# Scuttie/Few-Shot-Prompt-Learning-for-Vision-Language-Models-in-Imbalanced-Datasets

Hardware: AMD Instinct MI355X
Metric: CoCoOp ViT-B/16 16-shot train-step images/sec at 1/2/4/8 GPUs; eval images/sec (higher is better)
Workload: dtype fp32s

## Files before the change

few-shot-prompt-learning-for-vision-language-models-in-imbalanced-datasets_amd/_native.py:

```python
from __future__ import annotations

import ctypes
import hashlib
import os
import sys

_PKG = os.path.dirname(os.path.abspath(__file__))
LIB_PATH = os.environ.get("CLIPK_LIB") or os.path.join(_PKG, "libclipk.so")
_ROOT = os.path.dirname(_PKG)


def source_files():
    csrc = os.path.join(_PKG, "csrc")
    names = sorted(n for n in os.listdir(csrc) if n.endswith((".hip", ".h")) or n == "Makefile")
    rel = [("csrc/" + n, os.path.join(csrc, n)) for n in names]
    return rel + [("include/clipk.h", os.path.join(_ROOT, "include", "clipk.h"))]


def source_digest():
    h = hashlib.sha256()
    for rel, path in source_files():
        with open(path, "rb") as f:
            h.update(f"{hashlib.sha256(f.read()).hexdigest()}  {rel}\n".encode())
    return h.hexdigest()

F32, F16, BF16, F32S = 0, 1, 2, 3
PREFIX_CLS_GROUP0 = 1
PREFIX_SPLIT = 2
PREFIX_OUT_SPLIT = 4
F32S16 = 4
SPLIT_SCALE = 64.0
EPI_BIAS, EPI_BIAS_RES, EPI_BIAS_QGELU, EPI_DQGELU, EPI_NONE = 0, 1, 2, 3, 4
A_QGELU = 0x100
QGELU_DERIV = 0x200
OUT_SPLIT, A_SPLIT = 0x400, 0x800
ADAM_ADAM, ADAM_ADAMW, ADAM_AMSGRAD = 0, 1, 2
PROF_NONE, PROF_GEMM_FC, PROF_GEMM_ALL, PROF_ATTN, PROF_LN, PROF_GEMM_DGELU = 0, 1, 2, 3, 4, 5

_P = ctypes.c_void_p
_I = ctypes.c_int
_L = ctypes.c_long
_F = ctypes.c_float
_S = ctypes.c_size_t
_D = ctypes.c_double
_U = ctypes.c_uint

SIGNATURES = {
    "clipk_version": (ctypes.c_char_p, []),
    "clipk_source_digest": (ctypes.c_char_p, []),
    "clipk_strerror": (ctypes.c_char_p, [_I]),
    "clipk_device_arch_ok": (_I, []),
    "clipk_gemm": (_I, [_I, _I, _I, _I, _I, _I, _P, _I, _P, _I, _P, _P, _I, _P, _I, _P, _P, _I, _I, _P]),
    "clipk_gemm_auto_splits": (_I, [_I, _I, _I, _I]),
    "clipk_gemm_splitk_ws_bytes": (_S, [_I, _I, _I]),
    "clipk_gemm_splitk": (_I, [_I, _I, _I, _I, _I, _I, _P, _I, _P, _I, _P, _P, _I, _P, _I, _P, _I, _P, _S, _P]),
    "clipk_gemm_set_config": (_I, [_I]),
    "clipk_split_pack": (_I, [_I, _I, _P, _I, _P, _P]),
    "clipk_split_lo_zero": (_I, [_I, _I, _P, _P, _P]),
    "clipk_split_hi16": (_I, [_I, _I, _P, _P, _P]),
    "clipk_gemm_ln": (_I, [_I, _I, _I, _I, _I, _P, _I, _P, _I, _P, _P, _I, _P, _I, _P, _P, _P, _P, _P]),
    "clipk_ln_stats_merge": (_I, [_I, _I, _P, _P, _P, _P, _P]),
    "clipk_gemm_ln_merge_fused": (_I, [_I, _I, _I, _I]),
    "clipk_gemm_split_tile_rows": (_I, [_I, _I, _I, _I, _I]),
    "clipk_gemm_t256_cost": (_D, [_I, _I, _I]),
    "clipk_gemm_ln_stats_split": (_I, [_I, _I, _I, _I, _I, _P, _I, _P, _I, _P, _P, _I, _P, _I, _P, _P, _P, _P]),
    "clipk_gemm_ln_gamma": (_I, [_I, _I, _I, _I, _I, _P, _I, _P, _I, _P, _P, _I, _P, _P, _P, _P, _P]),
    "clipk_gemm_ln_merge": (_I, [_I, _I, _I, _I, _I, _P, _I, _P, _I, _P, _P, _I, _P, _P, _P, _P, _P, _P, _P]),
    "clipk_image_resample": (_I, [_I, _I, _I, _P, _P, _P, _P, _P, _P, _I, _P, _P]),
    "clipk_gemm_stamps": (_I, [_P, _S]),
    "clipk_layernorm_fwd": (_I, [_I, _I, _I, _P, _I, _P, _P, _P, _P, _I, _P, _P, _P]),
    "clipk_layernorm_bwd": (_I, [_I, _I, _I, _P, _I, _P, _I, _P, _P, _P, _P, _P, _I, _P, _P, _I, _P, _I, _P]),
    "clipk_layernorm_fwd_x": (_I, [_I, _I, _I, _I, _P, _I, _P, _P, _P, _P, _I, _P, _P, _P]),
    "clipk_layernorm_bwd_x": (_I, [_I, _I, _I, _I, _P, _I, _P, _I, _P, _P, _P, _P, _P, _I, _P, _P, _I, _P, _I, _P]),
    "clipk_layernorm_bwd_x2": (_I, [_I, _I, _I, _I, _P, _I, _P, _I, _P, _P, _P, _P, _P, _I, _I, _P, _P, _I, _P, _I, _P]),
    "clipk_attention_fwd": (_I, [_I, _I, _I, _I, _I, _P, _I, _P, _I, _P, _P]),
    "clipk_attention_bwd": (_I, [_I, _I, _I, _I, _I, _I, _P, _I, _P, _I, _P, _I, _P, _P, _I, _P]),
    "clipk_im2col": (_I, [_I, _I, _I, _I, _I, _P, _P, _P]),
    "clipk_vit_embed_ln": (_I, [_I, _I, _I, _P, _P, _P, _P, _P, _P, _P]),
    "clipk_prompt_assemble": (_I, [_I, _I, _I, _I, _P, _P, _P, _L, _L, _P, _P, _P, _P]),
    "clipk_ctx_grad": (_I, [_I, _I, _I, _I, _I, _I, _P, _P, _P, _P]),
    "clipk_prompt_assemble_rows": (_I, [_I, _I, _I, _I, _I, _P, _P, _P, _P, _L, _L, _P, _P, _P, _P]),
    "clipk_ctx_grad_rows": (_I, [_I, _I, _I, _I, _P, _P, _P, _P, _P]),
    "clipk_ctx_bias_grad_rows": (_I, [_I, _I, _I, _I, _P, _P, _P, _P, _P, _P]),
    "clipk_attention_prefix_fwd": (_I, [_I, _I, _I, _I, _I, _P, _P, _I, _P, _I, _P, _I, _P, _P]),
    "clipk_attention_prefix_ws_bytes": (_S, [_I, _I, _I]),
    "clipk_attention_prefix_bwd": (_I, [_I, _I, _I, _I, _I, _I, _P, _P, _I, _P, _I, _P, _I, _P, _I, _P, _P,
                                        _I, _P, _S, _P]),
    "clipk_attention_prefix_fwd_ex": (_I, [_I, _I, _I, _I, _I, _P, _P, _I, _P, _I, _P, _I, _P, _I, _P]),
    "clipk_attention_prefix_bwd_ex": (_I, [_I, _I, _I, _I, _I, _I, _P, _P, _I, _P, _I, _P, _I, _P, _I, _P, _P,
                                           _I, _P, _S, _I, _P]),
    "clipk_cosine_logits_fwd": (_I, [_I, _I, _I, _I, _F, _P, _P, _P, _P, _P, _P]),
    "clipk_cosine_logits_bwd": (_I, [_I, _I, _I, _I, _F, _P, _P, _P, _P, _P, _P, _P]),
    "clipk_ce_loss": (_I, [_I, _I, _P, _P, _P, _F, _I, _F, _P, _P, _P]),
    "clipk_ce_loss_reduce": (_I, [_I, _I, _P, _P, _P, _F, _I, _F, _I, _P, _P, _P, _P]),
    "clipk_ce_loss_mix": (_I, [_I, _I, _P, _P, _P, _F, _P, _F, _I, _F, _I, _P, _P, _P, _P]),
    "clipk_mixup_images": (_I, [_I, _L, _P, _P, _P, _P, _F, _F, _P, _P]),
    "clipk_ntxent_ws_bytes": (_S, [_I, _I]),
    "clipk_ntxent_loss": (_I, [_I, _I, _P, _P, _F, _F, _P, _P, _P, _P, _P]),
# ... 123 lines not shown
```

few-shot-prompt-learning-for-vision-language-models-in-imbalanced-datasets_amd/csrc/attention.hip:

```cpp
#include "attn_common.h"

namespace clipk {

template <int LP, typename T>
__global__ __launch_bounds__(256) void attn_fwd_short(int nseq, int L, int H, int causal,
                                                      const T* __restrict__ qkv, int ldq,
                                                      T* __restrict__ out, int ldo,
                                                      float* __restrict__ lse) {
  constexpr int G = 64 / LP;
  constexpr int V = Vec16<T>::N;
  __shared__ CLIPK_LDS_ALIGN T sk[4][64 * 64];
  __shared__ CLIPK_LDS_ALIGN T sv[4][64 * 64];
  const int lane = threadIdx.x & 63, w = threadIdx.x >> 6;
  const int g = lane / LP, i = lane % LP;
  const int pair = (blockIdx.x * 4 + w) * G + g;
  const bool pair_ok = pair < nseq * H;
  const int s = pair_ok ? pair / H : 0, h = pair_ok ? pair % H : 0;
  const int W = H * 64;
  const bool row_ok = pair_ok && i < L;
  const size_t row = (size_t)s * L + (row_ok ? i : 0);
  const T* qp = qkv + row * ldq + h * 64;

  T* myk = &sk[w][lane * 64];
  T* myv = &sv[w][lane * 64];
// ... 416 lines not shown
      t8 pv;
#pragma unroll
      for (int j = 0; j < 8; ++j) pv[j] = (T)p[j];
      const s16x8 pb = __builtin_bit_cast(s16x8, pv);
#pragma unroll
      for (int t = 0; t < 4; ++t) {
        const s16x4 lo = tr_read(sV, kb + 4 * g4, 16 * t, lane), hi = tr_read(sV, kb + 16 + 4 * g4, 16 * t, lane);
        const s16x8 va = __builtin_shufflevector(lo, hi, 0, 1, 2, 3, 4, 5, 6, 7);
        o[t] = mfma32_t<T>(va, pb, o[t]);
      }
    }
  }
  const float lt = xsum4(l);
  const float inv = 1.0f / lt;
  if (qok) {
    T* op = out + (row0 + qr) * ldo + h * 64 + 4 * g4;
#pragma unroll
    for (int t = 0; t < 4; ++t)
      *reinterpret_cast<s16x4*>(op + 16 * t) = pack4<T>(o[t][0] * inv, o[t][1] * inv, o[t][2] * inv, o[t][3] * inv);
    if (lse && g4 == 0) lse[(row0 + qr) * H + h] = (m + __log2f(lt)) * 0.6931471805599453f;
  }
}

template <typename T, typename TG>
__device__ __forceinline__ float row_D(const TG* dor, const T* orow, bool ok, int g4) {
  float acc = 0.f;
  if (ok) {
#pragma unroll
    for (int kk = 0; kk < 2; ++kk) {
      float a[8], b[8];
      load16_f32<TG>(dor + 8 * g4 + 32 * kk, a);
      load16_f32<T>(orow + 8 * g4 + 32 * kk, b);
#pragma unroll
      for (int c = 0; c < 8; ++c) acc = fmaf(a[c], b[c], acc);
    }
  }
  acc += __shfl_xor(acc, 16, 64);
  acc += __shfl_xor(acc, 32, 64);
  return acc;
}

template <typename T, typename TG>
__global__ __launch_bounds__(256) void attn_bwd_long_kv(int nseq, int L, int H, int causal,
                                                        const T* __restrict__ qkv, int ldq,
                                                        const T* __restrict__ o_fwd, int ldof,
                                                        const TG* __restrict__ dout, int lddo,
// ... 347 lines not shown
    CLIPK_CHECK_LAUNCH();
    return CLIPK_OK;
  }
  auto go = [&](auto lp_tag) {
    constexpr int LP = decltype(lp_tag)::value;
    constexpr int G = 64 / LP;
    const int blocks = (pairs + G - 1) / G;
    hipLaunchKernelGGL((attn_bwd_short<LP, T, TG>), dim3(blocks), dim3(64), 0, st, nseq, L, H,
                       causal, (const T*)qkv, ldq, (const T*)ofwd, ldof, (const TG*)dout, lddo, lse,
                       (TG*)dqkv, lddq);
  };
  if (L <= 16) go(std::integral_constant<int, 16>{});
  else if (L <= 32) go(std::integral_constant<int, 32>{});
  else if (L <= 64) go(std::integral_constant<int, 64>{});
  else return CLIPK_ESHAPE;
  CLIPK_CHECK_LAUNCH();
  return CLIPK_OK;
}

}

using namespace clipk;

extern "C" int clipk_attention_fwd(int dtype, int nseq, int L, int heads, int causal,
                                   const void* qkv, int ldqkv, void* out, int ldo, float* lse,
                                   void* stream) {
  if (!qkv || !out) return CLIPK_EINVAL;
  if (nseq < 0 || L <= 0 || heads <= 0 || ldqkv < 3 * heads * 64 || ldo < heads * 64 || ldqkv % 8 ||
      ldo % 8)
    return CLIPK_ESHAPE;
  if (nseq == 0) return CLIPK_OK;
  hipStream_t st = (hipStream_t)stream;
  switch (dtype) {
    case CLIPK_F16: return launch_fwd<f16>(nseq, L, heads, causal, qkv, ldqkv, out, ldo, lse, st);
    case CLIPK_BF16: return launch_fwd<bf16>(nseq, L, heads, causal, qkv, ldqkv, out, ldo, lse, st);
    case CLIPK_F32: return launch_fwd<float>(nseq, L, heads, causal, qkv, ldqkv, out, ldo, lse, st);
    default: return CLIPK_EDTYPE;
  }
}

extern "C" int clipk_attention_bwd(int dtype, int grad_dtype, int nseq, int L, int heads,
                                    int causal, const void* qkv, int ldqkv, const void* ofwd,
                                    int ldof, const void* dout, int lddo, const float* lse,
                                    void* dqkv, int lddqkv, void* stream) {
  if (!qkv || !ofwd || !dout || !lse || !dqkv) return CLIPK_EINVAL;
  if (nseq < 0 || L <= 0 || heads <= 0 || ldqkv < 3 * heads * 64 || lddqkv < 3 * heads * 64 ||
      ldof < heads * 64 || lddo < heads * 64)
    return CLIPK_ESHAPE;
  if (nseq == 0) return CLIPK_OK;
  hipStream_t st = (hipStream_t)stream;
#define CLIPK_BWD(TT, TGG) \
  return launch_bwd<TT, TGG>(nseq, L, heads, causal, qkv, ldqkv, ofwd, ldof, dout, lddo, lse, dqkv, lddqkv, st)
  if (dtype == CLIPK_F16 && grad_dtype == CLIPK_BF16) CLIPK_BWD(f16, bf16);
  if (dtype == CLIPK_F16 && grad_dtype == CLIPK_F16) CLIPK_BWD(f16, f16);
  if (dtype == CLIPK_BF16 && grad_dtype == CLIPK_BF16) CLIPK_BWD(bf16, bf16);
  if (dtype == CLIPK_F32 && grad_dtype == CLIPK_F32) CLIPK_BWD(float, float);
#undef CLIPK_BWD
  return CLIPK_EDTYPE;
}
```

few-shot-prompt-learning-for-vision-language-models-in-imbalanced-datasets_amd/csrc/attention_prefix.hip:

```cpp
#include <cstdlib>

#include "attn_common.h"

namespace clipk {

constexpr int kValuChunkMin = 4;

static int chunk_env(const char* name, int def) {
  const char* e = getenv(name);
  const int v = e ? atoi(e) : def;
  return v >= 1 && v <= 16 ? v : def;
}
static int lds_slots();
static int fwd_chunk() { static int c = chunk_env("CLIPK_PREFIX_FWD_CHUNK", lds_slots() ? 4 : 8); return c; }
static int bwd_chunk() { static int c = chunk_env("CLIPK_PREFIX_BWD_CHUNK", 16); return c; }
static int prefix_num_cus() {
  static int n = 0;
  if (!n) {
    int dev = 0, v = 0;
    n = (hipGetDevice(&dev) == hipSuccess &&
         hipDeviceGetAttribute(&v, hipDeviceAttributeMultiprocessorCount, dev) == hipSuccess && v > 0)
            ? v
            : 256;
  }
// ... 919 lines not shown
          akp[d] = fmaf(dsp, a[d], akp[d]);
          avp[d] = fmaf(pp, b[d], avp[d]);
        }
      }
      if (qok) {
        if constexpr (OS) {
          st16x_split(dqkv + row * lddq + W + h * 64 + kSl * s, dk, s);
          st16x_split(dqkv + row * lddq + 2 * W + h * 64 + kSl * s, dv, s);
        } else {
          st16x(dqkv + row * lddq + W + h * 64 + kSl * s, dk);
          st16x(dqkv + row * lddq + 2 * W + h * 64 + kSl * s, dv);
        }
      }
    }
    lds_sync();
  }
  if (r < P) {
    float* pb = part + (((size_t)g * nchunk + k) * 16 + r) * (2 * W) + h * 64 + kSl * s;
    st16x(pb, akp);
    st16x(pb + W, avp);
  }
}

constexpr float kPScale = 4096.0f, kPInv = 1.0f / 4096.0f;

struct Parts8 { s16x8 hi[2], lo[2]; };

__device__ __forceinline__ void ld_frag32(const float* p, f32x4 (&x)[4]) {
#pragma unroll
  for (int i = 0; i < 4; ++i) x[i] = *reinterpret_cast<const f32x4*>(p + 16 * i);
}
__device__ __forceinline__ void split_frag(const f32x4 (&x)[4], Parts8& o) {
#pragma unroll
  for (int kk = 0; kk < 2; ++kk) {
    f16x8 h, l;
#pragma unroll
    for (int j = 0; j < 2; ++j)
#pragma unroll
      for (int e = 0; e < 4; ++e) {
        const float v = x[2 * kk + j][e];
        const f16 hh = (f16)v;
        h[4 * j + e] = hh;
        l[4 * j + e] = (f16)(v - (float)hh);
      }
    o.hi[kk] = __builtin_bit_cast(s16x8, h);
    o.lo[kk] = __builtin_bit_cast(s16x8, l);
  }
}
__device__ __forceinline__ void split_pack4(float a, float b, float c, float d, s16x4& hi, s16x4& lo) {
  float x[4] = {a, b, c, d};
  typedef f16 h4 __attribute__((ext_vector_type(4)));
  h4 h, l;
#pragma unroll
  for (int e = 0; e < 4; ++e) {
    asm volatile("" : "+v"(x[e]));
    h[e] = (f16)x[e];
    l[e] = (f16)(x[e] - (float)h[e]);
  }
  hi = __builtin_bit_cast(s16x4, h);
  lo = __builtin_bit_cast(s16x4, l);
}
__device__ __forceinline__ void st_parts(const Parts8& f, short* thi, short* tlo, int r16, int g4) {
#pragma unroll
  for (int i = 0; i < 4; ++i) {
    const int o = r16 * TRS + 16 * i + 4 * g4;
    const s16x8 h = f.hi[i >> 1], l = f.lo[i >> 1];
    const int b = 4 * (i & 1);
    *reinterpret_cast<s16x4*>(thi + o) = (s16x4){h[b], h[b + 1], h[b + 2], h[b + 3]};
    *reinterpret_cast<s16x4*>(tlo + o) = (s16x4){l[b], l[b + 1], l[b + 2], l[b + 3]};
  }
}
__device__ __forceinline__ f32x4 mfma32_s3(const Parts8& a, const Parts8& b, f32x4 c) {
#pragma unroll
  for (int kk = 0; kk < 2; ++kk) {
    c = mfma32_t<f16>(a.lo[kk], b.hi[kk], c);
    c = mfma32_t<f16>(a.hi[kk], b.lo[kk], c);
  }
#pragma unroll
  for (int kk = 0; kk < 2; ++kk) c = mfma32_t<f16>(a.hi[kk], b.hi[kk], c);
  return c;
}
__device__ __forceinline__ f32x4 mfma16_s3(s16x4 ah, s16x4 al, s16x4 bh, s16x4 bl, f32x4 c) {
  c = mfma16_t<f16>(al, bh, c);
  c = mfma16_t<f16>(ah, bl, c);
  return mfma16_t<f16>(ah, bh, c);
}
__device__ __forceinline__ void ld_prefix_parts(const float* p, bool ok, Parts8& o) {
  f32x4 x[4];
  ld_frag32(p, x);
#pragma unroll
  for (int i = 0; i < 4; ++i)
    if (!ok) x[i] = (f32x4){0.f, 0.f, 0.f, 0.f};
  split_frag(x, o);
}
template <bool OS>
__device__ __forceinline__ void store_acc16(float* rowp, const f32x4 v, int t, bool ok, int g4) {
  if constexpr (!OS) {
    if (ok) *reinterpret_cast<f32x4*>(rowp + 16 * t + 4 * g4) = v;
  } else {
    typedef uint32_t u32x2 __attribute__((ext_vector_type(2)));
    s16x4 h, l;
    split_pack4(v[0], v[1], v[2], v[3], h, l);
    const u32x2 hu = __builtin_bit_cast(u32x2, h), lu = __builtin_bit_cast(u32x2, l);
    const auto s0 = __builtin_amdgcn_permlane16_swap(hu[0], lu[0], false, false);
    const auto s1 = __builtin_amdgcn_permlane16_swap(hu[1], lu[1], false, false);
    if (ok)
      reinterpret_cast<u32x4*>(rowp + 16 * t + 8 * (g4 >> 1))[g4 & 1] =
          (u32x4){(uint32_t)s0[0], (uint32_t)s1[0], (uint32_t)s0[1], (uint32_t)s1[1]};
  }
}
template <bool OS>
__device__ __forceinline__ void store_acc64(float* rowp, const f32x4 (&a)[4], float scale, bool ok, int g4) {
#pragma unroll
  for (int t = 0; t < 4; ++t) store_acc16<OS>(rowp, a[t] * scale, t, ok, g4);
}

constexpr int kSplitFwdWpc = 12, kSplitBwdWpc = 8;

template <int WPB, bool OS>
__global__ __launch_bounds__(WPB * 64) void attn_prefix_fwd_split(
    int G, int P, int R, int ntiles, const int* __restrict__ tiles, const int* __restrict__ row_first, int H,
    int nchunk, int uc, const float* __restrict__ qkv, int ldq, float* __restrict__ out, int ldo,
    float* __restrict__ lse, int cls0) {
  __shared__ CLIPK_LDS_ALIGN short sm[WPB][4][16 * TRS];
  const int lane = threadIdx.x & 63, w = threadIdx.x >> 6;
  const int r16 = lane & 15, g4 = lane >> 4;
  const int wid = blockIdx.x * WPB + w;
  if (wid >= G * nchunk * H) return;
  const int h = wid % H, k = (wid / H) % nchunk, g = wid / (H * nchunk);
  const int W = H * 64;
  short* sVpH = sm[w][0];
  short* sVpL = sm[w][1];
  short* sVoH = sm[w][2];
  short* sVoL = sm[w][3];
  const size_t gR = (size_t)g * R;
  const float* qh = qkv + h * 64 + 4 * g4;
  const int u_begin = k * uc, u_end = min((k + 1) * uc, ntiles + 1);
  const int tab = load_tile_table(tiles, ntiles, u_begin, lane);

// ... 572 lines not shown
```

few-shot-prompt-learning-for-vision-language-models-in-imbalanced-datasets_amd/csrc/attn_common.h:

```cpp
#pragma once
#include "common.h"

namespace clipk {

constexpr float kScale = 0.125f;
typedef uint32_t u32x4 __attribute__((ext_vector_type(4)));

template <typename T>
__device__ __forceinline__ void load_row64(const T* p, float* out) {
  constexpr int V = Vec16<T>::N;
#pragma unroll
  for (int c = 0; c < 64 / V; ++c) load16_f32<T>(p + c * V, out + c * V);
}

template <typename T>
__device__ __forceinline__ void store_row64(T* p, const float* in) {
  constexpr int V = Vec16<T>::N;
#pragma unroll
  for (int c = 0; c < 64 / V; ++c) store16_f32<T>(p + c * V, in + c * V);
}

template <typename T>
__device__ __forceinline__ void load_cols8(const T* p, float* out) {
  constexpr int V = Vec16<T>::N;
// ... 192 lines not shown
#pragma unroll
  for (int s = 0; s < 4; s += 2)
#pragma unroll
    for (int dw = 0; dw < 2; ++dw) {
      const auto r = __builtin_amdgcn_permlane32_swap(d[s][dw], d[s + 1][dw], false, false);
      d[s][dw] = r[0];
      d[s + 1][dw] = r[1];
    }
#pragma unroll
  for (int s = 0; s < 4; s += 2)
#pragma unroll
    for (int dw = 0; dw < 2; ++dw) {
      const auto r = __builtin_amdgcn_permlane16_swap(d[s][dw], d[s + 1][dw], false, false);
      d[s][dw] = r[0];
      d[s + 1][dw] = r[1];
    }
  if (ok) {
    const int g4 = (threadIdx.x & 63) >> 4;
    *reinterpret_cast<u32x4*>(rowp + 8 * g4) = (u32x4){d[0][0], d[0][1], d[1][0], d[1][1]};
    *reinterpret_cast<u32x4*>(rowp + 32 + 8 * g4) = (u32x4){d[2][0], d[2][1], d[3][0], d[3][1]};
  }
}

}
```

few-shot-prompt-learning-for-vision-language-models-in-imbalanced-datasets_amd/csrc/encoder.hip:

```cpp
#include <vector>
#include <array>
#include <cstring>
#include <new>
#include <cstdlib>
#include <algorithm>

#include "common.h"

struct DeepPrompts {
  int n_deep = 0, n_ctx = 0, n_per = 0;
  const int* rows = nullptr;
  const float* prompts = nullptr;
  float* grads = nullptr;
};

struct clipk_encoder {
  int kind;
  int W, layers, heads, E, act, grad;
  int res, patch, Kp, Limg;
  std::vector<std::array<const void*, 16>> lw;
  std::array<const void*, 8> head;
  DeepPrompts deep;
  int prefix_input = 0;
  std::vector<std::array<const void*, 6>> fold;
// ... 291 lines not shown
    SeqShape s;
    s.rows = nseq * L; s.nout = nseq; s.nseq = nseq; s.L = L; s.causal = causal;
    return s;
  }
  static SeqShape prefix(int G, int C, int P, int R, int ntiles, const int* tiles, const int* row_first) {
    SeqShape s;
    s.rows = G * R; s.nout = G * C; s.packed = true; s.causal = 1;
    s.G = G; s.C = C; s.P = P; s.R = R; s.ntiles = ntiles; s.tiles = tiles; s.row_first = row_first;
    return s;
  }
  size_t part_bytes(int heads) const { return packed ? clipk_attention_prefix_ws_bytes(G, ntiles, heads) : 0; }
};

constexpr int kPrefixSplitFwd = 1, kPrefixSplitBwd = 2, kPrefixSplitDefault = kPrefixSplitFwd | kPrefixSplitBwd;
static int prefix_split_flag(const clipk_encoder* e, int dir) {
  const char* s = getenv("CLIPK_PREFIX_SPLIT_ATTN");
  const int on = s ? atoi(s) : kPrefixSplitDefault;
  return (on & dir) && e->split != 0 && e->act == CLIPK_F32 ? CLIPK_PREFIX_SPLIT : 0;
}
static bool prefix_split_bwd(const clipk_encoder* e, const SeqShape& sh, int gd) {
  return sh.packed && gd == CLIPK_F32 && prefix_split_flag(e, kPrefixSplitBwd) != 0;
}

static int attn_fwd(const clipk_encoder* e, const SeqShape& sh, const void* qkv, void* o, float* lse,
                    hipStream_t st, int pflags = 0) {
  const int W = e->W;
  if (sh.packed)
    return clipk_attention_prefix_fwd_ex(e->act, sh.G, sh.P, sh.R, sh.ntiles, sh.tiles, sh.row_first, e->heads,
                                         qkv, 3 * W, o, W, lse,
                                         pflags | prefix_split_flag(e, kPrefixSplitFwd) |
                                             (t_osplit ? CLIPK_PREFIX_OUT_SPLIT : 0), st);
  return clipk_attention_fwd(e->act, sh.nseq, sh.L, e->heads, sh.causal, qkv, 3 * W, o, W, lse, st);
}

static int attn_bwd(const clipk_encoder* e, const SeqShape& sh, const void* qkv, const void* o,
                    const void* dout, const float* lse, void* dqkv, void* part, hipStream_t st,
                    bool dqkv_split = false, int pflags = 0) {
  const int W = e->W;
  if (sh.packed)
    return clipk_attention_prefix_bwd_ex(e->act, dqkv_split ? CLIPK_F32S : e->grad, sh.G, sh.P, sh.R, sh.ntiles, sh.tiles, sh.row_first,
                                      e->heads, qkv, 3 * W, o, W, dout, W, lse, dqkv, 3 * W, part,
                                      sh.part_bytes(e->heads),
                                      pflags | (prefix_split_bwd(e, sh, e->grad) ? CLIPK_PREFIX_SPLIT : 0), st);
  return clipk_attention_bwd(e->act, e->grad, sh.nseq, sh.L, e->heads, sh.causal, qkv, 3 * W, o, W, dout, W,
                             lse, dqkv, 3 * W, st);
}

static int block_attn(const clipk_encoder* e, const std::array<const void*, 16>& w, const SeqShape& sh, int rd,
                      const void* X, void* xn, void* qkv, void* o, float* lse, float* m1, float* r1,
                      hipStream_t st, bool text, void* sk, size_t skb) {
  const int pg = text ? CLIPK_PROF_GEMM_ALL : CLIPK_PROF_NONE;
  const int W = e->W, rows = sh.rows, act = e->act;
  const double lnb = (double)rows * W * (esize(rd) + esize(act)) + (m1 ? 8.0 * rows : 0.0);
  {
    ProfScope ps(CLIPK_PROF_NONE, st, 0.0, text ? "text.ln_fwd" : "vit.ln_fwd", lnb);
// ... 54 lines not shown
static int gemm_ln(int act, int epi, int M, int N, int K, const void* A, const void* B, const float* bias,
                   const void* res, void* o, void* o2, float* stats, const float* colsum, const float* rnb,
                   hipStream_t st, int prof_cls, const char* site, const float* gamma = nullptr) {
  const double b = gemm_bytes(act, act, epi, M, N, K, o2 != nullptr, act) + (stats ? (double)M * (N / 64) * 8 : 0.0) +
                   (rnb ? 8.0 * M : 0.0) + (gamma ? 4.0 * K : 0.0);
  ProfScope ps(prof_cls, st, 2.0 * M * N * K, site, b);
  if (t_split && act == CLIPK_F32) act = t_split == 2 ? CLIPK_F32S16 : CLIPK_F32S;
  if (gamma) return clipk_gemm_ln_gamma(act, epi, M, N, K, A, K, B, K, bias, o, N, o2, colsum, rnb, gamma, st);
  return clipk_gemm_ln(act, epi, M, N, K, A, K, B, K, bias, res, N, o, N, o2, stats, colsum, rnb, st);
}
static int gemm_ln_split2(int epi, int M, int N, int K, const void* A, const void* B, const float* bias,
                          const void* res, void* o, float* stats, const float* gamma, void* xs, hipStream_t st,
                          int prof_cls, const char* site) {
  const double b = gemm_bytes(CLIPK_F32S16, CLIPK_F32, epi, M, N, K, false, CLIPK_F32) + (double)M * (N / 64) * 8 +
                   4.0 * M * N + 4.0 * N;
  ProfScope ps(prof_cls, st, 2.0 * M * N * K, site, b);
  return clipk_gemm_ln_stats_split(CLIPK_F32S16, epi, M, N, K, A, K, B, K, bias, res, N, o, N, stats, gamma, xs, st);
}
static bool ps_fold(const clipk_encoder* e) { return t_split == 2 && e->split == 2 && presplit_on(); }
static bool o_split_on(const clipk_encoder* e, const SeqShape& sh, bool fold) {
  const char* s = getenv("CLIPK_PRESPLIT_O");
  return (s ? atoi(s) != 0 : true) && fold && ps_fold(e) && sh.packed && e->lora.rank == 0 &&
         prefix_split_flag(e, kPrefixSplitFwd) != 0 && prefix_split_bwd(e, sh, e->grad);
}
static int ln_merge(int rows, int W, const float* lnst, float* m, float* r, float* rnb, hipStream_t st, bool text) {
  ProfScope ps(CLIPK_PROF_NONE, st, 0.0, text ? "text.ln_stats" : "vit.ln_stats", (double)rows * (W / 64) * 8 + 16.0 * rows);
  return clipk_ln_stats_merge(rows, W, lnst, m, r, rnb, st);
}
static int gemm_ln_merged(int act, int epi, int M, int N, int K, const void* A, const void* B, const float* bias,
                          void* o, void* o2, const float* lnst, const float* colsum, float* m, float* r,
                          float* rnb, hipStream_t st, int prof_cls, const char* site, bool text,
                          const float* gamma = nullptr) {
  if (t_split || act == CLIPK_F32 || !clipk_gemm_ln_merge_fused(act, M, N, K)) {
    TRY(ln_merge(M, K, lnst, m, r, rnb, st, text));
    return gemm_ln(act, epi, M, N, K, A, B, bias, nullptr, o, o2, nullptr, colsum, rnb, st, prof_cls, site, gamma);
  }
  const double b = gemm_bytes(act, act, epi, M, N, K, o2 != nullptr, act) + (double)M * (K / 64) * 8 + 16.0 * M;
  ProfScope ps(prof_cls, st, 2.0 * M * N * K, site, b);
  return clipk_gemm_ln_merge(act, epi, M, N, K, A, K, B, K, bias, o, N, o2, lnst, colsum, m, r, rnb, st);
}
static int block_attn_fold(const clipk_encoder* e, const std::array<const void*, 6>& f, const SeqShape& sh,
                           const void* X, void* qkv, void* o, float* lse, float* m1, float* r1, const float* lnst,
                           float* rnb, hipStream_t st, bool text, const float* gamma = nullptr,
                           const void* xs = nullptr) {
  const int W = e->W, rows = sh.rows, act = e->act;
  TRY(gemm_ln_merged(act, CLIPK_EPI_BIAS | (xs ? CLIPK_A_SPLIT : 0), rows, 3 * W, W, xs ? xs : X, f[0],
// ... 226 lines not shown
}

static int text_forward_impl(const clipk_encoder* e, const SeqShape& sh, const float* x0, const int* eot_rows,
                             float* txt, void* saved, size_t saved_bytes, void* ws, size_t ws_bytes,
                             hipStream_t st, const EncIO& io) {
  SplitScope split_scope(e);
  const bool save = saved != nullptr;
  TextBufs t = text_layout(e, sh.rows, sh.nout, saved, ws, save, io.rd);
  if (ws_bytes < t.ws_bytes || (save && saved_bytes < t.saved_bytes)) return CLIPK_EWORKSPACE;
  const int W = e->W, rows = sh.rows, rd = io.rd;
  const int pg = io.text ? CLIPK_PROF_GEMM_ALL : CLIPK_PROF_NONE;
  const void* cur = x0;
  if (save || rd != CLIPK_F32) {
    if (rd == CLIPK_F32) {
      TRY(clipk_rows_copy(W * 4, rows, x0, nullptr, t.X[0], nullptr, st));
    } else {
      TRY(clipk_cast(rd, (long)rows * W, x0, t.X[0], st));
    }
    cur = t.X[0];
  }
  const bool eotl = text_eot_last(sh);
  const int nl = e->layers, nout = sh.nout;
  const bool fold = ln_fold_on(e, io);
  t_osplit = io.text && o_split_on(e, sh, fold);
  if (save) e->o_saved_split = t_osplit;
  bool have_stats = false;
  bool xs_ready = false;
  for (int l = 0; l < nl; ++l) {
    void* Xo = t.X[l + 1];
    if (!save && Xo == cur) Xo = t.X[l];
    if (l >= 1) TRY(deep_inject(e, l, rd, const_cast<void*>(cur), st));
    const bool share0 = l == 0 && io.text && sh.G >= 2 && prefix_mode(e, sh);
    float* m1 = save ? t.mean1[l] : t.tm;
    float* r1 = save ? t.rstd1[l] : t.tr;
    float* m2 = save ? t.mean2[l] : t.tm;
    float* r2 = save ? t.rstd2[l] : t.tr;
    if (share0)
      TRY(block_attn_shared0(e, e->lw[l], sh, rd, cur, t.xn, t.qkv[l], t.o[l], t.lse[l], t.mean1[l], t.rstd1[l],
                             (int*)t.g, st));
    else if (fold && have_stats)
      TRY(block_attn_fold(e, e->fold[l], sh, cur, t.qkv[l], t.o[l], t.lse[l], m1, r1, t.lnst, t.rnb, st, io.text,
                          e->split == 2 ? (const float*)e->lw[l][0] : nullptr, xs_ready ? t.xn : nullptr));
    else
      TRY(block_attn(e, e->lw[l], sh, rd, cur, t.xn, t.qkv[l], t.o[l], t.lse[l], t.mean1[l], t.rstd1[l], st,
                     io.text, io.sk, io.skb));
    const bool compact = eotl && l == nl - 1;
    const void* xin = cur;
// ... 664 lines not shown
```

few-shot-prompt-learning-for-vision-language-models-in-imbalanced-datasets_amd/ops.py:

```python
from __future__ import annotations

import ctypes

import torch

from . import _native as N

DT = {torch.float32: N.F32, torch.float16: N.F16, torch.bfloat16: N.BF16}


def _stream():
    return ctypes.c_void_p(torch.cuda.current_stream().cuda_stream)


def _p(t):
    return None if t is None else ctypes.c_void_p(t.data_ptr())


def _need(t, name, dtype=None, cuda=True):
    if t is None:
        raise N.ClipkError(f"{name} is required")
    if cuda and not t.is_cuda:
        raise N.ClipkError(f"{name} must be a CUDA(HIP) tensor; no CPU path exists")
    if dtype is not None and t.dtype != dtype:
# ... 179 lines not shown
    _need(dy, "dy")
    R, W = dy.shape
    dx = torch.empty(R, W, device=dy.device, dtype=torch.float32)
    split = lp_dtype == "split"
    lp = (torch.empty(R, W, device=dy.device, dtype=torch.float32 if split else lp_dtype)
          if lp_dtype is not None else None)
    lpd = N.F32S if split else (DT[lp_dtype] if lp_dtype is not None else 0)
    _need(x, "x")
    N.call("clipk_layernorm_bwd_x", DT[x.dtype], DT[dy.dtype], R, W, _p(dy), W, _p(x), W, None, _p(w), _p(mean),
           _p(rstd), _p(dres), W, _p(dx), _p(lp), lpd, None, W, _stream())
    return (dx, lp) if lp is not None else dx


def layernorm_bwd_lp_(dy, x, w, mean, rstd, dres_lp, dx=None):
    _need(dy, "dy")
    _need(x, "x")
    _need(dres_lp, "dres_lp")
    R, W = dy.shape
    N.call("clipk_layernorm_bwd_x2", DT[x.dtype], DT[dy.dtype], R, W, _p(dy), W, _p(x), W, None, _p(w), _p(mean),
           _p(rstd), _p(dres_lp), DT[dres_lp.dtype], W, _p(dx), _p(dres_lp), DT[dres_lp.dtype], None, W, _stream())
    return dres_lp


def attention(qkv, nseq, L, heads, causal, lse=False):
    _need(qkv, "qkv")
    W = heads * 64
    out = torch.empty(nseq * L, W, device=qkv.device, dtype=qkv.dtype)
    l = torch.empty(nseq * L, heads, device=qkv.device) if lse else None
    N.call("clipk_attention_fwd", DT[qkv.dtype], nseq, L, heads, int(causal), _p(qkv), 3 * W, _p(out),
           W, _p(l), _stream())
    return (out, l) if lse else out


def attention_bwd(qkv, o, dout, lse, nseq, L, heads, causal, grad_dtype):
    W = heads * 64
    dqkv = torch.empty(nseq * L, 3 * W, device=qkv.device, dtype=grad_dtype)
    N.call("clipk_attention_bwd", DT[qkv.dtype], DT[grad_dtype], nseq, L, heads, int(causal), _p(qkv),
           3 * W, _p(o), W, _p(dout), W, _p(lse), _p(dqkv), 3 * W, _stream())
    return dqkv


def im2col(img, patch, Kp, out_dtype):
    _need(img, "image", torch.float32)
    B, _, R, _ = img.shape
    G = R // patch
    out = torch.empty(B * G * G, Kp, device=img.device, dtype=out_dtype)
    N.call("clipk_im2col", DT[out_dtype], B, R, patch, Kp, _p(img), _p(out), _stream())
    return out


def prompt_assemble(B, C, L, src_map, emb, ctx, ctx_sb, ctx_sc, bias, pos):
    W = emb.shape[-1]
    x0 = torch.empty(B * C * L, W, device=emb.device, dtype=torch.float32)
# ... 455 lines not shown
```

include/clipk.h:

```cpp
#ifndef CLIPK_H
#define CLIPK_H

#include <stddef.h>
#include <stdint.h>

#ifdef __cplusplus
extern "C" {
#endif

enum { CLIPK_F32 = 0, CLIPK_F16 = 1, CLIPK_BF16 = 2, CLIPK_F32S = 3, CLIPK_F32S16 = 4 };

enum {
  CLIPK_OK = 0,
  CLIPK_EINVAL = -1,
  CLIPK_ESHAPE = -2,
  CLIPK_EDTYPE = -3,
  CLIPK_EWORKSPACE = -4,
  CLIPK_ERANGE = -5,
  CLIPK_EHIP = -6
};

enum {
  CLIPK_EPI_BIAS = 0,
  CLIPK_EPI_BIAS_RES = 1,
// ... 68 lines not shown
                        const int* in_rows, const float* gamma, const float* beta,
                        void* out, int ldo, float* mean, float* rstd, void* stream);
int clipk_layernorm_fwd_x(int x_dtype, int out_dtype, int rows, int width, const void* x, int ldx,
                          const int* in_rows, const float* gamma, const float* beta,
                          void* out, int ldo, float* mean, float* rstd, void* stream);

int clipk_layernorm_bwd(int dy_dtype, int rows, int width, const void* dy, int lddy, const float* x, int ldx,
                        const int* x_rows, const float* gamma, const float* mean, const float* rstd,
                        const float* dres, int lddres, float* dx, void* dx_lp, int lp_dtype,
                        const int* out_rows, int ldo, void* stream);
int clipk_layernorm_bwd_x(int x_dtype, int dy_dtype, int rows, int width, const void* dy, int lddy,
                          const void* x, int ldx, const int* x_rows, const float* gamma,
                          const float* mean, const float* rstd, const float* dres, int lddres,
                          float* dx, void* dx_lp, int lp_dtype, const int* out_rows, int ldo,
                          void* stream);
int clipk_layernorm_bwd_x2(int x_dtype, int dy_dtype, int rows, int width, const void* dy, int lddy,
                           const void* x, int ldx, const int* x_rows, const float* gamma,
                           const float* mean, const float* rstd, const void* dres, int dres_dtype,
                           int lddres, float* dx, void* dx_lp, int lp_dtype, const int* out_rows,
                           int ldo, void* stream);

int clipk_attention_fwd(int dtype, int nseq, int L, int heads, int causal,
                        const void* qkv, int ldqkv, void* out, int ldo, float* lse, void* stream);

int clipk_attention_bwd(int dtype, int grad_dtype, int nseq, int L, int heads, int causal,
                        const void* qkv, int ldqkv, const void* ofwd, int ldof, const void* dout,
                        int lddo, const float* lse, void* dqkv, int lddqkv, void* stream);

int clipk_attention_prefix_fwd(int dtype, int G, int P, int R, int ntiles, const int* tiles,
                               const int* row_first, int heads, const void* qkv, int ldqkv, void* out,
                               int ldo, float* lse, void* stream);
size_t clipk_attention_prefix_ws_bytes(int G, int ntiles, int heads);
int clipk_attention_prefix_bwd(int dtype, int grad_dtype, int G, int P, int R, int ntiles,
                               const int* tiles, const int* row_first, int heads, const void* qkv,
                               int ldqkv, const void* ofwd, int ldof, const void* dout, int lddo,
                               const float* lse, void* dqkv, int lddqkv, void* ws, size_t ws_bytes,
                               void* stream);

enum { CLIPK_PREFIX_CLS_GROUP0 = 1, CLIPK_PREFIX_SPLIT = 2, CLIPK_PREFIX_OUT_SPLIT = 4 };
int clipk_attention_prefix_fwd_ex(int dtype, int G, int P, int R, int ntiles, const int* tiles,
                                  const int* row_first, int heads, const void* qkv, int ldqkv, void* out,
                                  int ldo, float* lse, int flags, void* stream);
int clipk_attention_prefix_bwd_ex(int dtype, int grad_dtype, int G, int P, int R, int ntiles,
                                  const int* tiles, const int* row_first, int heads, const void* qkv,
                                  int ldqkv, const void* ofwd, int ldof, const void* dout, int lddo,
                                  const float* lse, void* dqkv, int lddqkv, void* ws, size_t ws_bytes,
// ... 185 lines not shown
```

Before: 381.2.

## Add split-fp16 MFMA forward attention kernel for fp32 ViT encoder

Adds an fp32 attention forward kernel that splits Q, K, V and P into fp16 hi/lo parts and uses three fp16 MFMAs per product, replacing the fp32 path for the vision encoder when split mode is active. It can optionally write the output already split into hi/lo form, so the following out-projection GEMM can skip its own split step in non-saving passes. The aim is to move ViT attention onto matrix cores while keeping near-fp32 accuracy. The cost is extra MFMA work and some loss of precision relative to true fp32.

```diff
diff --git a/few-shot-prompt-learning-for-vision-language-models-in-imbalanced-datasets_amd/_native.py b/few-shot-prompt-learning-for-vision-language-models-in-imbalanced-datasets_amd/_native.py
--- a/few-shot-prompt-learning-for-vision-language-models-in-imbalanced-datasets_amd/_native.py
+++ b/few-shot-prompt-learning-for-vision-language-models-in-imbalanced-datasets_amd/_native.py
@@ -28,6 +28,8 @@
 PREFIX_CLS_GROUP0 = 1
 PREFIX_SPLIT = 2
 PREFIX_OUT_SPLIT = 4
+ATTN_SPLIT = 1
+ATTN_OUT_SPLIT = 2
 F32S16 = 4
 SPLIT_SCALE = 64.0
 EPI_BIAS, EPI_BIAS_RES, EPI_BIAS_QGELU, EPI_DQGELU, EPI_NONE = 0, 1, 2, 3, 4
@@ -74,6 +76,7 @@
     "clipk_layernorm_bwd_x": (_I, [_I, _I, _I, _I, _P, _I, _P, _I, _P, _P, _P, _P, _P, _I, _P, _P, _I, _P, _I, _P]),
     "clipk_layernorm_bwd_x2": (_I, [_I, _I, _I, _I, _P, _I, _P, _I, _P, _P, _P, _P, _P, _I, _I, _P, _P, _I, _P, _I, _P]),
     "clipk_attention_fwd": (_I, [_I, _I, _I, _I, _I, _P, _I, _P, _I, _P, _P]),
+    "clipk_attention_fwd_ex": (_I, [_I, _I, _I, _I, _I, _P, _I, _P, _I, _P, _I, _P]),
     "clipk_attention_bwd": (_I, [_I, _I, _I, _I, _I, _I, _P, _I, _P, _I, _P, _I, _P, _P, _I, _P]),
     "clipk_im2col": (_I, [_I, _I, _I, _I, _I, _P, _P, _P]),
     "clipk_vit_embed_ln": (_I, [_I, _I, _I, _P, _P, _P, _P, _P, _P, _P]),
diff --git a/few-shot-prompt-learning-for-vision-language-models-in-imbalanced-datasets_amd/csrc/attention.hip b/few-shot-prompt-learning-for-vision-language-models-in-imbalanced-datasets_amd/csrc/attention.hip
--- a/few-shot-prompt-learning-for-vision-language-models-in-imbalanced-datasets_amd/csrc/attention.hip
+++ b/few-shot-prompt-learning-for-vision-language-models-in-imbalanced-datasets_amd/csrc/attention.hip
@@ -462,6 +462,162 @@
   }
 }
 
+template <bool OS>
+__global__ __launch_bounds__(256) void attn_fwd_split(int nseq, int L, int H, int causal,
+                                                      const float* __restrict__ qkv, int ldq,
+                                                      float* __restrict__ out, int ldo,
+                                                      float* __restrict__ lse) {
+  __shared__ CLIPK_LDS_ALIGN short sKh[64 * TRS];
+  __shared__ CLIPK_LDS_ALIGN short sKl[64 * TRS];
+  __shared__ CLIPK_LDS_ALIGN short sVh[64 * TRS];
+  __shared__ CLIPK_LDS_ALIGN short sVl[64 * TRS];
+  constexpr float kLog2e = 1.4426950408889634f;
+  const int tid = threadIdx.x, lane = tid & 63, w = tid >> 6;
+  const int r16 = lane & 15, g4 = lane >> 4;
+  const int h = blockIdx.y, s = blockIdx.z;
+  const int W = H * 64;
+  const size_t row0 = (size_t)s * L;
+  const int q0 = blockIdx.x * 64 + w * 16;
+  const int qr = q0 + r16;
+  const bool qok = qr < L;
+  s16x8 qh[2], ql[2];
+  {
+    const float* qp = qkv + (row0 + (qok ? qr : 0)) * ldq + h * 64 + 8 * g4;
+#pragma unroll
+    for (int kk = 0; kk < 2; ++kk) {
+      f32x4 x[2];
+#pragma unroll
+      for (int c = 0; c < 2; ++c)
+        x[c] = qok ? *reinterpret_cast<const f32x4*>(qp + 32 * kk + 4 * c) : (f32x4){0.f, 0.f, 0.f, 0.f};
+      f16x8 hh, ll;
+#pragma unroll
+      for (int c = 0; c < 2; ++c)
+#pragma unroll
+        for (int e = 0; e < 4; ++e) {
+          f16 ph, pl;
+          split_parts(x[c][e] * kScale, ph, pl);
+          hh[4 * c + e] = ph;
+          ll[4 * c + e] = pl;
+        }
+      qh[kk] = __builtin_bit_cast(s16x8, hh);
+      ql[kk] = __builtin_bit_cast(s16x8, ll);
+    }
+  }
+
+  f32x4 o[4];
+#pragma unroll
+  for (int t = 0; t < 4; ++t) o[t] = (f32x4){0.f, 0.f, 0.f, 0.f};
+  float m = -INFINITY, l = 0.f;
+  const int qmax = min(L, (int)(blockIdx.x + 1) * 64) - 1;
+  const int kend = causal ? qmax + 1 : L;
+  f32x4 rk[2][2], rv[2][2];
+  auto fetch = [&](int k0) {
+#pragma unroll
+    for (int it = 0; it < 2; ++it) {
+      const int kr = k0 + it * 32 + (tid >> 3), ch = tid & 7;
+      const bool ok = kr < L;
+      const float* base = qkv + (row0 + (ok ? kr : 0)) * ldq + h * 64 + ch * 8;
+#pragma unroll
+      for (int c = 0; c < 2; ++c) {
+        rk[it][c] = ok ? *reinterpret_cast<const f32x4*>(base + W + 4 * c) : (f32x4){0.f, 0.f, 0.f, 0.f};
+        rv[it][c] = ok ? *reinterpret_cast<const f32x4*>(base + 2 * W + 4 * c) : (f32x4){0.f, 0.f, 0.f, 0.f};
+      }
+    }
+  };
+  auto st_split = [&](const f32x4& a, const f32x4& b, short* thi, short* tlo) {
+    const unsigned h01 = __builtin_bit_cast(unsigned, (f16x2){(f16)a[0], (f16)a[1]});
+    const unsigned h23 = __builtin_bit_cast(unsigned, (f16x2){(f16)a[2], (f16)a[3]});
+    const unsigned h45 = __builtin_bit_cast(unsigned, (f16x2){(f16)b[0], (f16)b[1]});
+    const unsigned h67 = __builtin_bit_cast(unsigned, (f16x2){(f16)b[2], (f16)b[3]});
+    unsigned l01, l23, l45, l67;
+    split_lo4(a[0], a[1], a[2], a[3], h01, h23, l01, l23);
+    split_lo4(b[0], b[1], b[2], b[3], h45, h67, l45, l67);
+    *reinterpret_cast<u32x4*>(thi) = (u32x4){h01, h23, h45, h67};
+    *reinterpret_cast<u32x4*>(tlo) = (u32x4){l01, l23, l45, l67};
+  };
+  fetch(0);
+  for (int k0 = 0; k0 < kend; k0 += 64) {
+    __syncthreads();
+#pragma unroll
+    for (int it = 0; it < 2; ++it) {
+      const int off = (it * 32 + (tid >> 3)) * TRS + (tid & 7) * 8;
+      st_split(rk[it][0], rk[it][1], sKh + off, sKl + off);
+      st_split(rv[it][0], rv[it][1], sVh + off, sVl + off);
+    }
+    __syncthreads();
+    if (k0 + 64 < kend) fetch(k0 + 64);
+    const int npair = min(2, (kend - k0 + 31) / 32);
+    for (int pc = 0; pc < npair; ++pc) {
+      const int kb = pc * 32;
+      const int kabs = k0 + kb;
+      if (causal && kabs > q0 + 15) break;
+      float sv[8];
+#pragma unroll
+      for (int sub = 0; sub < 2; ++sub) {
+        f32x4 sb = {0.f, 0.f, 0.f, 0.f}, ss = {0.f, 0.f, 0.f, 0.f};
+#pragma unroll
+        for (int kk = 0; kk < 2; ++kk) {
+          const int off = (kb + sub * 16 + r16) * TRS + 8 * g4 + 32 * kk;
+          const s16x8 kh = *reinterpret_cast<const s16x8*>(sKh + off);
+          const s16x8 kl = *reinterpret_cast<const s16x8*>(sKl + off);
+          ss = mfma32_t<f16>(kl, qh[kk], ss);
+          ss = mfma32_t<f16>(kh, ql[kk], ss);
+          sb = mfma32_t<f16>(kh, qh[kk], sb);
+        }
+#pragma unroll
+        for (int r = 0; r < 4; ++r) sv[4 * sub + r] = (sb[r] + ss[r]) * kLog2e;
+      }
+      if (kabs + 32 > L || (causal && kabs + 31 > q0)) {
+#pragma unroll
+        for (int j = 0; j < 8; ++j) {
+          const int key = kabs + (j < 4 ? 4 * g4 + j : 16 + 4 * g4 + j - 4);
+          if (key >= L || (causal && key > qr)) sv[j] = -INFINITY;
+        }
+      }
+      float mx = sv[0];
+#pragma unroll
+      for (int j = 1; j < 8; ++j) mx = fmaxf(mx, sv[j]);
+      mx = xmax4(mx);
+      const float mn = fmaxf(m, mx);
+      const float msafe = mn == -INFINITY ? 0.f : mn;
+      float p[8], ps = 0.f;
+#pragma unroll
+      for (int j = 0; j < 8; ++j) {
+        p[j] = __builtin_amdgcn_exp2f(sv[j] - msafe);
+        ps += p[j];
+      }
+      if (__builtin_amdgcn_ballot_w64(mn > m) != 0) {
+        const float corr = __builtin_amdgcn_exp2f(m - msafe);
+        l *= corr;
+#pragma unroll
+        for (int t = 0; t < 4; ++t) o[t] *= corr;
+      }
+      l += ps;
+      m = mn;
+      s16x4 ph[2], pl[2];
+#pragma unroll
+      for (int c = 0; c < 2; ++c)
+        split_pack4(p[4 * c] * kPScale, p[4 * c + 1] * kPScale, p[4 * c + 2] * kPScale, p[4 * c + 3] * kPScale,
+                    ph[c], pl[c]);
+      const s16x8 pbh = __builtin_shufflevector(ph[0], ph[1], 0, 1, 2, 3, 4, 5, 6, 7);
+      const s16x8 pbl = __builtin_shufflevector(pl[0], pl[1], 0, 1, 2, 3, 4, 5, 6, 7);
+#pragma unroll
+      for (int t = 0; t < 4; ++t) {
+        const s16x8 vh = __builtin_shufflevector(tr_read(sVh, kb + 4 * g4, 16 * t, lane),
+                                                 tr_read(sVh, kb + 16 + 4 * g4, 16 * t, lane), 0, 1, 2, 3, 4, 5, 6, 7);
+        const s16x8 vl = __builtin_shufflevector(tr_read(sVl, kb + 4 * g4, 16 * t, lane),
+                                                 tr_read(sVl, kb + 16 + 4 * g4, 16 * t, lane), 0, 1, 2, 3, 4, 5, 6, 7);
+        o[t] = mfma32_t<f16>(vl, pbh, o[t]);
+        o[t] = mfma32_t<f16>(vh, pbl, o[t]);
+        o[t] = mfma32_t<f16>(vh, pbh, o[t]);
+      }
+    }
+  }
+  const float lt = xsum4(l);
+  store_acc64<OS>(out + (row0 + (qok ? qr : 0)) * ldo + h * 64, o, kPInv / lt, qok, g4);
+  if (lse && g4 == 0 && qok) lse[(row0 + qr) * H + h] = (m + __log2f(lt)) * 0.6931471805599453f;
+}
+
 template <typename T, typename TG>
 __device__ __forceinline__ float row_D(const TG* dor, const T* orow, bool ok, int g4) {
   float acc = 0.f;
@@ -855,21 +1011,46 @@
 
 using namespace clipk;
 
-extern "C" int clipk_attention_fwd(int dtype, int nseq, int L, int heads, int causal,
-                                   const void* qkv, int ldqkv, void* out, int ldo, float* lse,
-                                   void* stream) {
+static int attention_fwd_call(int dtype, int nseq, int L, int heads, int causal, const void* qkv, int ldqkv,
+                              void* out, int ldo, float* lse, int flags, void* stream) {
   if (!qkv || !out) return CLIPK_EINVAL;
+  if (flags & ~(CLIPK_ATTN_SPLIT | CLIPK_ATTN_OUT_SPLIT)) return CLIPK_EINVAL;
+  if (flags && dtype != CLIPK_F32) return CLIPK_EINVAL;
+  if ((flags & CLIPK_ATTN_OUT_SPLIT) && (!(flags & CLIPK_ATTN_SPLIT) || ldo % 8 || L <= 16)) return CLIPK_EINVAL;
   if (nseq < 0 || L <= 0 || heads <= 0 || ldqkv < 3 * heads * 64 || ldo < heads * 64 || ldqkv % 8 ||
       ldo % 8)
     return CLIPK_ESHAPE;
   if (nseq == 0) return CLIPK_OK;
   hipStream_t st = (hipStream_t)stream;
+  if ((flags & CLIPK_ATTN_SPLIT) && L > 16) {
+    dim3 grid((L + 63) / 64, heads, nseq);
+    if (flags & CLIPK_ATTN_OUT_SPLIT)
+      hipLaunchKernelGGL((attn_fwd_split<true>), grid, dim3(256), 0, st, nseq, L, heads, causal, (const float*)qkv,
+                         ldqkv, (float*)out, ldo, lse);
+    else
+      hipLaunchKernelGGL((attn_fwd_split<false>), grid, dim3(256), 0, st, nseq, L, heads, causal, (const float*)qkv,
+                         ldqkv, (float*)out, ldo, lse);
+    CLIPK_CHECK_LAUNCH();
+    return CLIPK_OK;
+  }
   switch (dtype) {
     case CLIPK_F16: return launch_fwd<f16>(nseq, L, heads, causal, qkv, ldqkv, out, ldo, lse, st);
     case CLIPK_BF16: return launch_fwd<bf16>(nseq, L, heads, causal, qkv, ldqkv, out, ldo, lse, st);
     case CLIPK_F32: return launch_fwd<float>(nseq, L, heads, causal, qkv, ldqkv, out, ldo, lse, st);
     default: return CLIPK_EDTYPE;
   }
+}
+
+extern "C" int clipk_attention_fwd(int dtype, int nseq, int L, int heads, int causal,
+                                   const void* qkv, int ldqkv, void* out, int ldo, float* lse,
+                                   void* stream) {
+  return attention_fwd_call(dtype, nseq, L, heads, causal, qkv, ldqkv, out, ldo, lse, 0, stream);
+}
+
+extern "C" int clipk_attention_fwd_ex(int dtype, int nseq, int L, int heads, int causal,
+                                      const void* qkv, int ldqkv, void* out, int ldo, float* lse,
+                                      int flags, void* stream) {
+  return attention_fwd_call(dtype, nseq, L, heads, causal, qkv, ldqkv, out, ldo, lse, flags, stream);
 }
 
 extern "C" int clipk_attention_bwd(int dtype, int grad_dtype, int nseq, int L, int heads,
diff --git a/few-shot-prompt-learning-for-vision-language-models-in-imbalanced-datasets_amd/csrc/attention_prefix.hip b/few-shot-prompt-learning-for-vision-language-models-in-imbalanced-datasets_amd/csrc/attention_prefix.hip
--- a/few-shot-prompt-learning-for-vision-language-models-in-imbalanced-datasets_amd/csrc/attention_prefix.hip
+++ b/few-shot-prompt-learning-for-vision-language-models-in-imbalanced-datasets_amd/csrc/attention_prefix.hip
@@ -965,7 +965,6 @@
   }
 }
 
-constexpr float kPScale = 4096.0f, kPInv = 1.0f / 4096.0f;
 
 struct Parts8 { s16x8 hi[2], lo[2]; };
 
@@ -990,19 +989,6 @@
     o.lo[kk] = __builtin_bit_cast(s16x8, l);
   }
 }
-__device__ __forceinline__ void split_pack4(float a, float b, float c, float d, s16x4& hi, s16x4& lo) {
-  float x[4] = {a, b, c, d};
-  typedef f16 h4 __attribute__((ext_vector_type(4)));
-  h4 h, l;
-#pragma unroll
-  for (int e = 0; e < 4; ++e) {
-    asm volatile("" : "+v"(x[e]));
-    h[e] = (f16)x[e];
-    l[e] = (f16)(x[e] - (float)h[e]);
-  }
-  hi = __builtin_bit_cast(s16x4, h);
-  lo = __builtin_bit_cast(s16x4, l);
-}
 __device__ __forceinline__ void st_parts(const Parts8& f, short* thi, short* tlo, int r16, int g4) {
 #pragma unroll
   for (int i = 0; i < 4; ++i) {
@@ -1036,28 +1022,6 @@
     if (!ok) x[i] = (f32x4){0.f, 0.f, 0.f, 0.f};
   split_frag(x, o);
 }
-template <bool OS>
-__device__ __forceinline__ void store_acc16(float* rowp, const f32x4 v, int t, bool ok, int g4) {
-  if constexpr (!OS) {
-    if (ok) *reinterpret_cast<f32x4*>(rowp + 16 * t + 4 * g4) = v;
-  } else {
-    typedef uint32_t u32x2 __attribute__((ext_vector_type(2)));
-    s16x4 h, l;
-    split_pack4(v[0], v[1], v[2], v[3], h, l);
-    const u32x2 hu = __builtin_bit_cast(u32x2, h), lu = __builtin_bit_cast(u32x2, l);
-    const auto s0 = __builtin_amdgcn_permlane16_swap(hu[0], lu[0], false, false);
-    const auto s1 = __builtin_amdgcn_permlane16_swap(hu[1], lu[1], false, false);
-    if (ok)
-      reinterpret_cast<u32x4*>(rowp + 16 * t + 8 * (g4 >> 1))[g4 & 1] =
-          (u32x4){(uint32_t)s0[0], (uint32_t)s1[0], (uint32_t)s0[1], (uint32_t)s1[1]};
-  }
-}
-template <bool OS>
-__device__ __forceinline__ void store_acc64(float* rowp, const f32x4 (&a)[4], float scale, bool ok, int g4) {
-#pragma unroll
-  for (int t = 0; t < 4; ++t) store_acc16<OS>(rowp, a[t] * scale, t, ok, g4);
-}
-
 constexpr int kSplitFwdWpc = 12, kSplitBwdWpc = 8;
 
 template <int WPB, bool OS>
diff --git a/few-shot-prompt-learning-for-vision-language-models-in-imbalanced-datasets_amd/csrc/attn_common.h b/few-shot-prompt-learning-for-vision-language-models-in-imbalanced-datasets_amd/csrc/attn_common.h
--- a/few-shot-prompt-learning-for-vision-language-models-in-imbalanced-datasets_amd/csrc/attn_common.h
+++ b/few-shot-prompt-learning-for-vision-language-models-in-imbalanced-datasets_amd/csrc/attn_common.h
@@ -238,4 +238,41 @@
   }
 }
 
-}
+constexpr float kPScale = 4096.0f, kPInv = 1.0f / 4096.0f;
+
+__device__ __forceinline__ void split_pack4(float a, float b, float c, float d, s16x4& hi, s16x4& lo) {
+  float x[4] = {a, b, c, d};
+  typedef f16 h4 __attribute__((ext_vector_type(4)));
+  h4 h, l;
+#pragma unroll
+  for (int e = 0; e < 4; ++e) {
+    asm volatile("" : "+v"(x[e]));
+    h[e] = (f16)x[e];
+    l[e] = (f16)(x[e] - (float)h[e]);
+  }
+  hi = __builtin_bit_cast(s16x4, h);
+  lo = __builtin_bit_cast(s16x4, l);
+}
+template <bool OS>
+__device__ __forceinline__ void store_acc16(float* rowp, const f32x4 v, int t, bool ok, int g4) {
+  if constexpr (!OS) {
+    if (ok) *reinterpret_cast<f32x4*>(rowp + 16 * t + 4 * g4) = v;
+  } else {
+    typedef uint32_t u32x2 __attribute__((ext_vector_type(2)));
+    s16x4 h, l;
+    split_pack4(v[0], v[1], v[2], v[3], h, l);
+    const u32x2 hu = __builtin_bit_cast(u32x2, h), lu = __builtin_bit_cast(u32x2, l);
+    const auto s0 = __builtin_amdgcn_permlane16_swap(hu[0], lu[0], false, false);
+    const auto s1 = __builtin_amdgcn_permlane16_swap(hu[1], lu[1], false, false);
+    if (ok)
+      reinterpret_cast<u32x4*>(rowp + 16 * t + 8 * (g4 >> 1))[g4 & 1] =
+          (u32x4){(uint32_t)s0[0], (uint32_t)s1[0], (uint32_t)s0[1], (uint32_t)s1[1]};
+  }
+}
+template <bool OS>
+__device__ __forceinline__ void store_acc64(float* rowp, const f32x4 (&a)[4], float scale, bool ok, int g4) {
+#pragma unroll
+  for (int t = 0; t < 4; ++t) store_acc16<OS>(rowp, a[t] * scale, t, ok, g4);
+}
+
+}
diff --git a/few-shot-prompt-learning-for-vision-language-models-in-imbalanced-datasets_amd/csrc/encoder.hip b/few-shot-prompt-learning-for-vision-language-models-in-imbalanced-datasets_amd/csrc/encoder.hip
--- a/few-shot-prompt-learning-for-vision-language-models-in-imbalanced-datasets_amd/csrc/encoder.hip
+++ b/few-shot-prompt-learning-for-vision-language-models-in-imbalanced-datasets_amd/csrc/encoder.hip
@@ -337,6 +337,11 @@
   return sh.packed && gd == CLIPK_F32 && prefix_split_flag(e, kPrefixSplitBwd) != 0;
 }
 
+static int attn_split_flag(const clipk_encoder* e) {
+  const char* s = getenv("CLIPK_VIT_SPLIT_ATTN");
+  return (s ? atoi(s) != 0 : true) && e->split != 0 && e->act == CLIPK_F32 ? CLIPK_ATTN_SPLIT : 0;
+}
+
 static int attn_fwd(const clipk_encoder* e, const SeqShape& sh, const void* qkv, void* o, float* lse,
                     hipStream_t st, int pflags = 0) {
   const int W = e->W;
@@ -345,7 +350,8 @@
                                          qkv, 3 * W, o, W, lse,
                                          pflags | prefix_split_flag(e, kPrefixSplitFwd) |
                                              (t_osplit ? CLIPK_PREFIX_OUT_SPLIT : 0), st);
-  return clipk_attention_fwd(e->act, sh.nseq, sh.L, e->heads, sh.causal, qkv, 3 * W, o, W, lse, st);
+  return clipk_attention_fwd_ex(e->act, sh.nseq, sh.L, e->heads, sh.causal, qkv, 3 * W, o, W, lse,
+                                attn_split_flag(e) | (t_osplit ? CLIPK_ATTN_OUT_SPLIT : 0), st);
 }
 
 static int attn_bwd(const clipk_encoder* e, const SeqShape& sh, const void* qkv, const void* o,
@@ -446,6 +452,11 @@
   const char* s = getenv("CLIPK_PRESPLIT_O");
   return (s ? atoi(s) != 0 : true) && fold && ps_fold(e) && sh.packed && e->lora.rank == 0 &&
          prefix_split_flag(e, kPrefixSplitFwd) != 0 && prefix_split_bwd(e, sh, e->grad);
+}
+static bool vit_o_split_on(const clipk_encoder* e, const SeqShape& sh, bool fold, bool save) {
+  const char* s = getenv("CLIPK_PRESPLIT_O");
+  return (s ? atoi(s) != 0 : true) && !save && fold && ps_fold(e) && !sh.packed && sh.L > 16 && e->lora.rank == 0 &&
+         attn_split_flag(e) != 0;
 }
 static int ln_merge(int rows, int W, const float* lnst, float* m, float* r, float* rnb, hipStream_t st, bool text) {
   ProfScope ps(CLIPK_PROF_NONE, st, 0.0, text ? "text.ln_stats" : "vit.ln_stats", (double)rows * (W / 64) * 8 + 16.0 * rows);
@@ -718,7 +729,7 @@
   const bool eotl = text_eot_last(sh);
   const int nl = e->layers, nout = sh.nout;
   const bool fold = ln_fold_on(e, io);
-  t_osplit = io.text && o_split_on(e, sh, fold);
+  t_osplit = io.text ? o_split_on(e, sh, fold) : vit_o_split_on(e, sh, fold, save);
   if (save) e->o_saved_split = t_osplit;
   bool have_stats = false;
   bool xs_ready = false;
diff --git a/few-shot-prompt-learning-for-vision-language-models-in-imbalanced-datasets_amd/ops.py b/few-shot-prompt-learning-for-vision-language-models-in-imbalanced-datasets_amd/ops.py
--- a/few-shot-prompt-learning-for-vision-language-models-in-imbalanced-datasets_amd/ops.py
+++ b/few-shot-prompt-learning-for-vision-language-models-in-imbalanced-datasets_amd/ops.py
@@ -225,13 +225,13 @@
     return dres_lp
 
 
-def attention(qkv, nseq, L, heads, causal, lse=False):
+def attention(qkv, nseq, L, heads, causal, lse=False, flags=0):
     _need(qkv, "qkv")
     W = heads * 64
     out = torch.empty(nseq * L, W, device=qkv.device, dtype=qkv.dtype)
     l = torch.empty(nseq * L, heads, device=qkv.device) if lse else None
-    N.call("clipk_attention_fwd", DT[qkv.dtype], nseq, L, heads, int(causal), _p(qkv), 3 * W, _p(out),
-           W, _p(l), _stream())
+    N.call("clipk_attention_fwd_ex", DT[qkv.dtype], nseq, L, heads, int(causal), _p(qkv), 3 * W, _p(out),
+           W, _p(l), int(flags), _stream())
     return (out, l) if lse else out
 
 
diff --git a/include/clipk.h b/include/clipk.h
--- a/include/clipk.h
+++ b/include/clipk.h
@@ -114,6 +114,10 @@
 
 int clipk_attention_fwd(int dtype, int nseq, int L, int heads, int causal,
                         const void* qkv, int ldqkv, void* out, int ldo, float* lse, void* stream);
+enum { CLIPK_ATTN_SPLIT = 1, CLIPK_ATTN_OUT_SPLIT = 2 };
+int clipk_attention_fwd_ex(int dtype, int nseq, int L, int heads, int causal,
+                           const void* qkv, int ldqkv, void* out, int ldo, float* lse, int flags,
+                           void* stream);
 
 int clipk_attention_bwd(int dtype, int grad_dtype, int nseq, int L, int heads, int causal,
                         const void* qkv, int ldqkv, const void* ofwd, int ldof, const void* dout,
```

Result: faster. 386.6 (median of 6 runs) (+1.4%).
